# balisujohn/tortoise.cpp

Measured on AMD Instinct MI355X. Metric: audio-seconds/sec end-to-end (AR+diffusion+vocoder), 16 cands x 80 steps, higher is better.
Workload: dtype f16 MFMA inputs / f32 accumulate (diffusion, vocoder convs); f32 weights, f16 KV (AR)

## Files before the change

### tortoise.cpp_amd/csrc/api.cpp

```cpp
#include "common.h"
#include <sched.h>
#include <cctype>
#include <algorithm>
#include <chrono>
#include <fstream>
#include <new>

namespace tts {
int ar_begin(tts_ctx *, const int32_t *, int, const float *, int, int);
int ar_begin_groups(tts_ctx *, const int32_t *, const int *, int, const float *, int n_voices, const int *voice_of, const int *, int);
int ar_latents_group(tts_ctx *, int, const int32_t *, int, float *);
int ar_prefill(tts_ctx *, float *);
int ar_step(tts_ctx *, const int32_t *, int, float *, int mode);
const int32_t *ar_host_lists(tts_ctx *);
const float *ar_fetch_logits_row(tts_ctx *, int);
int ar_batch(const tts_ctx *);
int ar_latents(tts_ctx *, const int32_t *, int, int, float *);
int ar_layers(const tts_ctx *);
float *ar_host_logits(tts_ctx *);
int diff_layers(const tts_ctx *);
int diff_forward(tts_ctx *, const float *, int, const float *, int, int, float *);
int diff_sample(tts_ctx *, const float *, const int32_t *, int, int, const float *, int, float *);
int diff_sample_voices(tts_ctx *, const float *, const int32_t *, int, const float *, int, const int32_t *, int, const float *, int, float *);
int voc_run(tts_ctx *, const float *, const int32_t *, int, const float *, int, float *);
// ... 112 lines not shown
  for (hipEvent_t e : c->ev_pool) (void)hipEventDestroy(e);
  if (c->ev0) (void)hipEventDestroy(c->ev0);
  if (c->ev1) (void)hipEventDestroy(c->ev1);
  if (c->stream) (void)hipStreamDestroy(c->stream);
  if (c->load_stream) (void)hipStreamDestroy(c->load_stream);
  delete c;
}

int tts_version(void) { return TTS_API_VERSION; }

const char *tts_last_error(const tts_ctx *c) { return c ? c->err.c_str() : "no context (no HIP device?)"; }

int tts_set_option(tts_ctx *c, const char *key, double value) {
  if (!c || !key) return TTS_ERR_ARG;
  std::string k(key);
  if (k == "gn_eps") c->gn_eps = (float)value;
  else if (k == "ggml_lut") c->ggml_lut = value != 0;
  else if (k.rfind("prof_only:", 0) == 0) {
    if (value != 0) c->prof_filter.push_back(k.substr(10));
    else c->prof_filter.clear();
  }
  else if (k == "device_topk") c->device_topk = value != 0;
  else if (k == "sampler_threads") {
    if (c->sampler_pool) { sampler_pool_free(c->sampler_pool); c->sampler_pool = nullptr; }
    c->sampler_threads = value < 0 ? -1 : (int)value;
  }
  else if (k == "share_uncond") c->share_uncond = value != 0;
  else if (k == "prof_stride") c->prof_stride = value < 1 ? 1 : (int)value;
  else if (k == "diff_graph") c->diff_graph = value != 0;
  else if (k == "dec_f32_mfma") c->dec_f32_mfma = value != 0;
  else if (k == "attn_f32") c->attn_f32 = value != 0;
  else if (k == "attn_proj_f16") c->attn_proj_f16 = value != 0;
  else if (k == "proj_dual_b") c->proj_dual_b = value != 0;
  else if (k == "lc_attn_f32") c->lc_attn_f32 = value != 0;
  else if (k == "latency_mode") c->latency_mode = value != 0;
  else if (k == "fp16_check") c->fp16_check = value != 0;
  else if (k == "rng_fast_normal") c->rng_fast_normal = value != 0;
  else if (k == "noise_pipeline") c->noise_pipeline = value != 0;
  else if (k == "load_device_pack") c->load_device_pack = value != 0;
  else if (k == "load_threads") c->load_threads = value < 0 ? 0 : value > 64 ? 64 : (int)value;
  else if (k == "attn_q64") c->attn_q64 = value < 0 ? 0 : value > 2 ? 2 : (int)value;
  else if (k == "hoist_integrator") c->hoist_integrator = value < 0 ? 0 : (int)value;
  else if (k == "attn_f32_drop") c->attn_f32_drop = (int)value & 7;
  else if (k == "ar_weights") {
    if (value != 0 && value != 1 && value != 2) return fail(c, TTS_ERR_ARG, "ar_weights: 0 (f32), 1 (fp16) or 2 (fp8 e4m3)");
    c->ar_weights = (int)value;
  }
  else if (k == "prof_eager_every") c->prof_eager_every = value < 1 ? 1 : (int)value;
  else if (k == "stream_cus") {
    if (c->device < 0) return fail(c, TTS_ERR_HIP, "host-only context: no stream");
    if (c->ar || c->diff || c->voc || c->clvp || c->venc || c->dcond) return fail(c, TTS_ERR_STATE, "stream_cus must be set before the models are loaded");
    (void)hipSetDevice(c->device);
    hipDeviceProp_t prop;
    if (hipGetDeviceProperties(&prop, c->device) != hipSuccess) return fail(c, TTS_ERR_HIP, "hipGetDeviceProperties failed");
    const int xcds = 8, per_xcd = prop.multiProcessorCount / xcds, n = (int)(value < 0 ? -value : value);
    if (prop.multiProcessorCount % xcds || per_xcd > 32 || n >= per_xcd) return fail(c, TTS_ERR_ARG, "stream_cus %d: the device has %d CUs per XCD", (int)value, per_xcd);
    hipStream_t s = nullptr;
    if (n == 0) {
      if (hipStreamCreate(&s) != hipSuccess) return fail(c, TTS_ERR_HIP, "hipStreamCreate failed");
    } else {
      uint32_t mask[8] = {0, 0, 0, 0, 0, 0, 0, 0};
      for (int slot = 0; slot < per_xcd; slot++)
        if ((slot < n) == (value > 0))
          for (int x = 0; x < xcds; x++) { const int bit = slot * xcds + x; mask[bit >> 5] |= 1u << (bit & 31); }
      if (hipExtStreamCreateWithCUMask(&s, (uint32_t)((per_xcd * xcds + 31) / 32), mask) != hipSuccess)
        return fail(c, TTS_ERR_HIP, "hipExtStreamCreateWithCUMask failed");
// ... 423 lines not shown
```

### tortoise.cpp_amd/csrc/common.h

```cpp
#pragma once
#include "../../include/tortoise_mi355x.h"
#include <hip/hip_runtime.h>
#include <cstdarg>
#include <cstdint>
#include <cstdio>
#include <cstring>
#include <functional>
#include <map>
#include <memory>
#include <random>
#include <algorithm>
#include <atomic>
#include <condition_variable>
#include <mutex>
#include <new>
#include <string>
#include <thread>
#include <vector>

namespace tts {

struct HostTensor {
  std::vector<float> data;
  int64_t ne[4] = {1, 1, 1, 1};
// ... 67 lines not shown
  int device = 0;
  hipStream_t stream = nullptr;
  hipStream_t load_stream = nullptr;
  int stream_cus = 0;
  std::string err;
  float gn_eps = 1e-6f;
  int ggml_lut = 0;
  std::mt19937 generator;
  std::uniform_real_distribution<float> distribution{0.0, 1.0};
  std::normal_distribution<double> normal_distribution{0.0, 1.0};
  uint32_t seed_value = 0;
  tts::ArState *ar = nullptr;
  tts::DiffState *diff = nullptr;
  tts::VocState *voc = nullptr;
  tts::ClvpState *clvp = nullptr;
  tts::VoiceEncState *venc = nullptr;
  tts::DiffCondEncState *dcond = nullptr;
  tts::Tokenizer *tok = nullptr;
  tts::SamplerPool *sampler_pool = nullptr;
  int device_topk = 1;
  int time_mlp_retries = 0;
  int topk_fallbacks = 0;
  int sampler_threads = -1;
  bool share_uncond = true;
  int rng_shard_offset = 0, rng_shard_total = 0;
  std::vector<int32_t> stop_schedule;
  std::vector<int32_t> ar_stopped;
  bool prof_on = false;
  std::vector<std::string> prof_filter;
  int prof_stride = 1;
  int ar_weights = 0;
  int dec_f32_mfma = 0;
  int attn_f32 = 0;
  int proj_dual_b = 1;
  int attn_f32_drop = 0;
  int lc_attn_f32 = 1;
  int attn_proj_f16 = 0;
  int fp16_check = 0;
  int64_t fp16_bad_weights[2] = {0, 0};
  void *fp16_counts = nullptr;
  int rng_fast_normal = 1;
  int noise_pipeline = 1;
  int load_device_pack = 1;
  int load_threads = 0;
  int attn_q64 = 0;
  int hoist_integrator = 1;
  int latency_mode = 0;
  bool capturing = false;
  int diff_graph = 1;
  int prof_eager_every = 8;
  std::map<std::string, tts::ProfEntry> prof;
  std::vector<hipEvent_t> ev_pool;
  hipEvent_t ev0 = nullptr, ev1 = nullptr;
};

namespace tts {

int fail(tts_ctx *ctx, int code, const char *fmt, ...);

void rng_normal_fill(tts_ctx *ctx, float *dst, int64_t n);

struct PinnedPool {
  explicit PinnedPool(size_t min_cap_ = (size_t)18 << 20, int max_bufs_ = 4) : min_cap(min_cap_), max_bufs(max_bufs_) {}
  size_t min_cap;
  int max_bufs, made = 0;
  std::mutex mu;
// ... 169 lines not shown
```

### tortoise.cpp_amd/csrc/diffusion.hip

```cpp
#include "common.h"
#include "gemm_f16.h"
#include <algorithm>
#include <chrono>
#include <cmath>

namespace tts {

static constexpr int C = 1024, NHEAD = 16, XTC = 128 ;
static constexpr int LAT_MAX_ROWS = 2048;
static constexpr int HOIST_MAX_ROWS = 16384;

__device__ __forceinline__ float silu_dev(float x, int lut) {
  if (lut == 1) {
    float xr = __half2float(__float2half_rn(x));
    return __half2float(__float2half_rn(xr / (1.0f + expf(-xr))));
  }
  if (lut == 2) return x / (1.0f + expf(-x));
  return x * __builtin_amdgcn_rcpf(1.0f + __builtin_amdgcn_exp2f(x * -1.44269504088896f));
}

__global__ __launch_bounds__(256) void gn_stats_kernel(const float *__restrict__ x, const int *__restrict__ seq_start,
                                                       const int *__restrict__ seq_len, float eps, float2 *__restrict__ stats) {
  __shared__ float sh[8];
  const int grp = blockIdx.x, s = blockIdx.y, T = seq_len[s];
// ... 626 lines not shown
  {
#pragma clang fp contract(off)
    const float frac = (var_c + 1) / 2;
    model_log_variance = frac * sc.min_log + (1 - frac) * sc.max_log;
    const float eps = (1 + sc.cfk) * eps_c - sc.cfk * eps_u;
    float x0 = sc.sqrt_recip * xv - sc.sqrt_recipm1 * eps;
    x0 = fminf(fmaxf(x0, -1.0f), 1.0f);
    mean = sc.coef1 * x0 + sc.coef2 * xv;
  }
  float outv = mean;
  if (!sc.is_last) {
    const float nz = noise ? noise[xi] : philox_normal(seed, stream0 + (uint32_t)s, step, (uint32_t)(ch * T + t));
    outv = (float)((double)mean + exp(0.5 * (double)model_log_variance) * (double)nz);
  }
  x[xi] = outv;
}

__global__ void philox_fill_kernel(float *__restrict__ x, int64_t n, uint64_t seed, uint32_t stream, uint32_t step) {
  int64_t i = (int64_t)blockIdx.x * blockDim.x + threadIdx.x;
  if (i < n) x[i] = philox_normal(seed, stream, step, (uint32_t)i);
}

__global__ void rows_to_ct_kernel(const float *__restrict__ net, int row0, int T, int nch, int ld, float *__restrict__ out) {
  int i = blockIdx.x * blockDim.x + threadIdx.x;
  if (i < nch * T) {
    int ch = i / T, t = i - ch * T;
    out[i] = net[(size_t)(row0 + t) * ld + ch];
  }
}

struct AttnDev {
  float *norm_g, *norm_b, *qkv_b, *proj_b, *bias_tab;
  __half *qkv_w, *proj_w;
  __half *proj_w_split;
  float proj_alpha;
};
struct ResDev { float *in_g, *in_b, *in_bias, *emb_w, *emb_b, *out_g, *out_b, *out_bias; __half *in_w, *out_w; };

struct Layout {
  int ns = 0, rows = 0;
  std::vector<int> start, len;
  DevBuf d_row_seq, d_row_t, d_start, d_len, d_chunk_seq;
  int build(tts_ctx *ctx, const std::vector<int> &lens) {
    has_seq_step = false; ss_step_stride = 0;
    ns = (int)lens.size();
    len = lens;
    start.resize(ns);
    int r = 8;
    for (int s = 0; s < ns; s++) { start[s] = r; r = (r + lens[s] + 1 + 7) & ~7; }
    rows = (r + 127) & ~127;
    std::vector<int> rs(rows, -1), rt(rows, 0);
    for (int s = 0; s < ns; s++)
      for (int t = 0; t < lens[s]; t++) { rs[start[s] + t] = s; rt[start[s] + t] = t; }
    TTS_HIP(ctx, d_row_seq.reserve(rows * 4)); TTS_HIP(ctx, d_row_t.reserve(rows * 4));
    TTS_HIP(ctx, d_start.reserve(ns * 4)); TTS_HIP(ctx, d_len.reserve(ns * 4));
    TTS_HIP(ctx, hipMemcpy(d_row_seq.p, rs.data(), rows * 4, hipMemcpyHostToDevice));
    TTS_HIP(ctx, hipMemcpy(d_row_t.p, rt.data(), rows * 4, hipMemcpyHostToDevice));
    TTS_HIP(ctx, hipMemcpy(d_start.p, start.data(), ns * 4, hipMemcpyHostToDevice));
    TTS_HIP(ctx, hipMemcpy(d_len.p, len.data(), ns * 4, hipMemcpyHostToDevice));
    std::vector<int> cs(rows / 8, -1);
    for (int s = 0; s < ns; s++)
      for (int t = 0; t < lens[s]; t++) cs[(start[s] + t) >> 3] = s;
    TTS_HIP(ctx, d_chunk_seq.reserve(rows / 8 * 4));
    TTS_HIP(ctx, hipMemcpy(d_chunk_seq.p, cs.data(), rows / 8 * 4, hipMemcpyHostToDevice));
    return TTS_OK;
  }
  int max_len() const { return len.empty() ? 0 : *std::max_element(len.begin(), len.end()); }
  DevBuf d_seq_step;
  int ss_step_stride = 0;
  bool has_seq_step = false;
// ... 87 lines not shown
  if (!latent2048) return fail(ctx, TTS_ERR_ARG, "null latent");
  TTS_HIP(ctx, hipMemcpyAsync(ctx->diff->cond_latent, latent2048, (size_t)2 * C * 4, hipMemcpyHostToDevice, ctx->stream));
  TTS_HIP(ctx, hipStreamSynchronize(ctx->stream));
  return TTS_OK;
}

namespace {
struct Loader {
  tts_ctx *ctx; DiffState *st; const WeightFile &wf; std::map<std::string, bool> used; std::mutex mu; PinnedPool pin{(size_t)9 << 20, 4};
  const HostTensor *get(const std::string &name, int64_t nelem) {
    auto it = wf.t.find(name);
    if (it == wf.t.end()) { fail(ctx, TTS_ERR_FORMAT, "tensor '%s' missing from diffusion model file", name.c_str()); return nullptr; }
    if (it->second.nelem() != nelem) {
      fail(ctx, TTS_ERR_FORMAT, "tensor '%s' has wrong size in model file: got %lld, expected %lld", name.c_str(),
           (long long)it->second.nelem(), (long long)nelem);
      return nullptr;
    }
    { std::lock_guard<std::mutex> lk(mu); used[name] = true; }
    return &it->second;
  }
  template <class T> int put(const std::vector<T> &h, T **dst) {
    void *p = nullptr;
    TTS_HIP(ctx, hipMalloc(&p, h.size() * sizeof(T)));
    { std::lock_guard<std::mutex> lk(mu); st->owned.push_back(p); }
    TTS_HIP(ctx, pin.upload(p, h.data(), h.size() * sizeof(T), ctx->load_stream));
    *dst = (T *)p;
    return TTS_OK;
  }
  int f32(const std::string &name, int64_t n, float **dst) {
    const HostTensor *t = get(name, n);
    if (!t) return TTS_ERR_FORMAT;
    return put(t->data, dst);
  }
  int conv16(const std::string &name, int cout, int cin, int k, int cout_pad, int cin_pad, __half **dst) {
    const HostTensor *t = get(name, (int64_t)cout * cin * k);
    if (!t) return TTS_ERR_FORMAT;
    std::vector<__half> h((size_t)cout_pad * k * cin_pad, __float2half(0.f));
    const float *w = t->data.data();
    for (int co = 0; co < cout; co++)
      for (int ci = 0; ci < cin; ci++)
        for (int tap = 0; tap < k; tap++)
          h[(size_t)co * k * cin_pad + (size_t)tap * cin_pad + ci] = __float2half_rn(w[((size_t)co * cin + ci) * k + tap]);
    return put(h, dst);
  }
  int attn(const std::string &p, AttnDev &a) {
    int r;
    if ((r = f32(p + ".norm.weight", C, &a.norm_g))) return r;
    if ((r = f32(p + ".norm.bias", C, &a.norm_b))) return r;
    if ((r = conv16(p + ".qkv.weight", 3 * C, C, 1, 3 * C, C, &a.qkv_w))) return r;
    if ((r = f32(p + ".qkv.bias", 3 * C, &a.qkv_b))) return r;
    if ((r = conv16(p + ".proj_out.weight", C, C, 1, C, C, &a.proj_w))) return r;
    {
      const HostTensor *t = get(p + ".proj_out.weight", (int64_t)C * C);
      std::vector<__half> sp((size_t)C * 2 * C);
      float amax = 0.f;
      for (float v : t->data) amax = std::max(amax, std::fabs(v));
      if (!std::isfinite(amax)) { fail(ctx, TTS_ERR_FORMAT, "tensor '%s.proj_out.weight' holds a non-finite value", p.c_str()); return TTS_ERR_FORMAT; }
      int e = 14;
      while (e > -14 && std::ldexp(amax, e) >= 30000.0f) e--;
      const float scale = std::ldexp(1.0f, e);
      a.proj_alpha = 1.0f / scale;
      for (int n = 0; n < C; n++)
        for (int k = 0; k < C; k++) {
          const float w = t->data[(size_t)n * C + k] * scale;
          const __half hi = __float2half_rn(w);
          sp[(size_t)n * 2 * C + k] = hi;
          sp[(size_t)n * 2 * C + C + k] = __float2half_rn(w - __half2float(hi));
        }
      long long bad[2] = {0, 0};
      for (const __half &h : sp) {
        const float v = std::fabs(__half2float(h));
        if (!(v <= 65504.0f)) bad[0]++;
        else if (v > 60000.0f) bad[1]++;
      }
      if (bad[0] | bad[1]) { std::lock_guard<std::mutex> lk(mu); ctx->fp16_bad_weights[0] += bad[0]; ctx->fp16_bad_weights[1] += bad[1]; }
      if ((r = put(sp, &a.proj_w_split))) return r;
    }
    if ((r = f32(p + ".proj_out.bias", C, &a.proj_b))) return r;
    const HostTensor *t = get(p + ".relative_pos_embeddings.relative_attention_bias.weight", 32 * 16);
    if (!t) return TTS_ERR_FORMAT;
    std::vector<float> tab(16 * 128);
    for (int h = 0; h < 16; h++)
      for (int sgn = 0; sgn < 2; sgn++)
        for (int d = 0; d < 64; d++) {
          int bucket = sgn ? rel_bucket(0, d) : rel_bucket(d, 0);
          if (d == 0) bucket = rel_bucket(0, 0);
          tab[h * 128 + sgn * 64 + d] = t->data[(size_t)bucket * 16 + h] * 8.0f;
        }
    return put(tab, &a.bias_tab);
  }
  int res(const std::string &p, ResDev &w) {
    int r;
    if ((r = f32(p + ".in_layers.0.weight", C, &w.in_g))) return r;
    if ((r = f32(p + ".in_layers.0.bias", C, &w.in_b))) return r;
    if ((r = conv16(p + ".in_layers.2.weight", C, C, 1, C, C, &w.in_w))) return r;
    if ((r = f32(p + ".in_layers.2.bias", C, &w.in_bias))) return r;
    if ((r = f32(p + ".emb_layers.1.weight", 2 * C * C, &w.emb_w))) return r;
    if ((r = f32(p + ".emb_layers.1.bias", 2 * C, &w.emb_b))) return r;
    if ((r = f32(p + ".out_layers.0.weight", C, &w.out_g))) return r;
    if ((r = f32(p + ".out_layers.0.bias", C, &w.out_b))) return r;
    if ((r = conv16(p + ".out_layers.3.weight", C, C, 3, C, C, &w.out_w))) return r;
    if ((r = f32(p + ".out_layers.3.bias", C, &w.out_bias))) return r;
    return TTS_OK;
  }
};
}

int diff_load(tts_ctx *ctx, const char *path) {
  ctx->fp16_bad_weights[0] = ctx->fp16_bad_weights[1] = 0;
  WeightFile wf;
  std::string err;
  int rc = read_weight_file(path, wf, err);
  if (rc != TTS_OK) return fail(ctx, rc, "diffusion_model_load: %s", err.c_str());
  std::unique_ptr<DiffState> st(new DiffState());
  Loader ld{ctx, st.get(), wf, {}};
  while (wf.has("latent_conditioner." + std::to_string(st->n_lc + 1) + ".norm.weight")) st->n_lc++;
  while (wf.has("conditioning_timestep_integrator." + std::to_string(st->n_integ) + ".resblk.in_layers.0.weight")) st->n_integ++;
  while (wf.has("layers." + std::to_string(st->n_main) + ".resblk.in_layers.0.weight")) st->n_main++;
  while (wf.has("layers." + std::to_string(st->n_main + st->n_tail) + ".in_layers.0.weight")) st->n_tail++;
  st->lc_attn.resize(st->n_lc);
  st->integ_res.resize(st->n_integ); st->integ_attn.resize(st->n_integ);
  st->main_res.resize(st->n_main); st->main_attn.resize(st->n_main);
  st->tail_res.resize(st->n_tail);
  std::vector<std::function<int()>> jobs;
  DiffState *S = st.get();
#define J(x) jobs.emplace_back([&ld, S]() -> int { (void)S; return (x); })
  J(ld.f32("diffusion_conditioning_latent", 2 * C, &S->cond_latent));
  J(ld.f32("unconditioned_embedding", C, &S->uncond_emb));
// ... 77 lines not shown
  int64_t dev[2] = {0, 0};
  if (ctx->fp16_counts) {
    TTS_HIP(ctx, hipStreamSynchronize(ctx->stream));
    TTS_HIP(ctx, hipMemcpy(dev, ctx->fp16_counts, 16, hipMemcpyDeviceToHost));
  }
  counts[0] = dev[0] + ctx->fp16_bad_weights[0];
  counts[1] = dev[1] + ctx->fp16_bad_weights[1];
  return TTS_OK;
}

static int gemm(tts_ctx *ctx, const char *fam, GemmArgs &g, const Layout &lay, int n_valid = 0, int k_valid = 0) {
  double mv = 0;
  for (int l : lay.len) mv += l;
  static const bool log_shapes = getenv("TTS_GEMM_LOG") != nullptr;
  if (log_shapes) fprintf(stderr, "gemm M=%d N=%d K=%dx%d mode=%d resid=%d\n", g.M, g.N, g.nseg, g.kseg, g.mode, g.resid != nullptr);
  if (!strcmp(fam, "diff_gemm")) {
    if (g.mode == GEMM_OUT_QKV) fam = "diff_gemm_qkv";
    else if (gemm_is_conv3(g) && g.N == C && g.kseg == C) fam = g.resid ? "diff_gemm_k3r" : "diff_gemm_k3";
    else if (g.nseg == 1 && g.N == C && g.kseg == C && g.mode == GEMM_OUT_F32) fam = g.resid ? "diff_gemm_k1r" : "diff_gemm_k1";
    else if (g.custom_w && g.N == C && g.kseg == C && g.mode == GEMM_OUT_F32_SCALED && g.resid) fam = "diff_gemm_k1r";
    else fam = "diff_gemm_misc";
  }
  ProfScope ps(ctx, fam, 2.0 * mv * (n_valid ? n_valid : g.N) * (k_valid ? k_valid : g.nseg * g.kseg));
  TTS_HIP(ctx, launch_gemm_f16(g, ctx->stream));
  if (ctx->fp16_check) {
    if (gemm_mode_qkv(g.mode)) {
      CHECK(fp16_check(ctx, g.outH, (size_t)g.M * g.ldh));
      CHECK(fp16_check(ctx, g.outVt, (size_t)(g.N / 3) * g.ldvt));
    } else if (g.mode == GEMM_OUT_F16) CHECK(fp16_check(ctx, g.outH, (size_t)g.M * g.ldh));
  }
  return TTS_OK;
}

static GemmArgs gemm_base(const Layout &lay, const __half *A, int lda, int nseg, int kseg, const __half *W, int N,
                          const float *bias) {
  GemmArgs g{};
  for (int i = 0; i < 3; i++) { g.A[i] = A; g.row_off[i] = 0; }
  if (nseg == 3) { g.row_off[0] = -1; g.row_off[1] = 0; g.row_off[2] = 1; }
  g.nseg = nseg; g.kseg = kseg; g.lda = lda; g.W = W; g.M = lay.rows; g.N = N; g.bias = bias;
  g.row_seq = lay.d_row_seq.as<int>();
  return g;
}

static int gn_stats(tts_ctx *ctx, const Layout &lay, Work &wk, const float *x) {
  ProfScope ps(ctx, "diff_gn_stats");
  gn_stats_kernel<<<dim3(32, lay.ns), 256, 0, ctx->stream>>>(x, lay.d_start.as<int>(), lay.d_len.as<int>(), ctx->gn_eps,
                                                             wk.stats.as<float2>());
  TTS_HIP(ctx, hipGetLastError());
  return TTS_OK;
}
template <int NT, int NJ>
__global__ __launch_bounds__(NT) void gn_reg_kernel(const float *__restrict__ x, const int *__restrict__ seq_start,
                                                    const int *__restrict__ seq_len, int rows_total, int ns, float eps,
                                                    const float *__restrict__ g, const float *__restrict__ b,
                                                    const float *__restrict__ ss, int do_silu, int lut, __half *__restrict__ y,
                                                    const char *__restrict__ pf0, int pf0_lines, const char *__restrict__ pf1, int pf1_lines,
                                                    const int *__restrict__ seq_step, int ss_step_stride) {
  constexpr int NW = NT / 64, SWEEP = NT / 8;
  __shared__ float sh[2][NW];
  __shared__ unsigned pf_sink[NW][64];
  const int bid = blockIdx.y * 32 + blockIdx.x, nbk = ns * 32, item = (bid & 7) * (nbk >> 3) + (bid >> 3);
  const int s = item >> 5, grp = item & 31;
  const int T = seq_len[s], r0 = seq_start[s];
  const int q = threadIdx.x & 7, c = grp * 32 + q * 4, t0 = threadIdx.x >> 3;
  const float *base = x + (size_t)r0 * C + c;
  float4 v[NJ];
// ... 157 lines not shown
      const __half2 p0 = __floats2half2_rn(e[0], e[1]), p1 = __floats2half2_rn(e[2], e[3]);
      uint2 o;
      o.x = *(const unsigned *)&p0;
      o.y = *(const unsigned *)&p1;
      *(uint2 *)(y + (size_t)(r0 + r) * C + c) = o;
    }
  };
  if (!do_silu) apply(std::integral_constant<int, 0>{});
  else if (lut == 0) apply(std::integral_constant<int, 1>{});
  else if (lut == 1) apply(std::integral_constant<int, 2>{});
  else apply(std::integral_constant<int, 3>{});
  if (pf0_lines | pf1_lines) asm volatile("s_waitcnt vmcnt(0)" ::: "memory");
}

static int gn(tts_ctx *ctx, const DiffState *st, const Layout &lay, const float *x, const long long *st_x, const float *g, const float *b, const float *ss, int do_silu,
              __half *y, const void *wa = nullptr, size_t wa_bytes = 0, const void *wb = nullptr, size_t wb_bytes = 0) {
  if (!st_x) {
    CHECK(gn_fused(ctx, lay, x, g, b, ss, do_silu, y, wa, wa_bytes, wb, wb_bytes));
    return fp16_check(ctx, y, (size_t)lay.rows * C);
  }
  {
    ProfScope ps(ctx, "diff_gn_apply");
    const int silu_mode = ctx->ggml_lut ? 1 : ctx->attn_f32 ? 2 : 0;
    gn_apply_kernel<<<lay.rows / 4, 256, 0, ctx->stream>>>(x, lay.d_chunk_seq.as<int>(), lay.d_start.as<int>(), lay.d_len.as<int>(), st_x, (int)st->gn_stripe_ll, ctx->gn_eps, g, b,
                                                            ss, do_silu, silu_mode, y, (const char *)wa, (int)(wa_bytes >> 7), (const char *)wb, (int)(wb_bytes >> 7),
                                                            lay.seq_step_ptr(), lay.ss_step_stride);
    TTS_HIP(ctx, hipGetLastError());
  }
  return fp16_check(ctx, y, (size_t)lay.rows * C);
}

static int res_in_layers(tts_ctx *ctx, const DiffState *st, const Layout &lay, Work &wk, const float *x, const ResDev &w, float *H,
                         const long long *st_x = nullptr, long long *st_h_out = nullptr) {
  CHECK(gn(ctx, st, lay, x, st_x, w.in_g, w.in_b, nullptr, 1, wk.A16(), w.in_w, (size_t)C * C * 2));
  DBG_SUM("res.in gn", wk.A16(), (size_t)lay.rows * C * 2);
  GemmArgs g = gemm_base(lay, wk.A16(), C, 1, C, w.in_w, C, w.in_bias);
  g.mode = st_h_out ? GEMM_OUT_F32_STATS : GEMM_OUT_F32; g.outF = H; g.ldo = C; g.resid = nullptr;
  g.st_out = st_h_out; g.st_stripe_ll = (int)st->gn_stripe_ll; g.chunk_seq = lay.d_chunk_seq.as<int>();
  CHECK(gemm(ctx, "diff_gemm", g, lay));
  DBG_SUM("res.in conv", H, (size_t)lay.rows * C * 4);
  return TTS_OK;
}

static int attention_block(tts_ctx *ctx, DiffState *st, const Layout &lay, Work &wk, float *X, const AttnDev &w, bool force_ref = false) {
  const bool f32 = ctx->attn_f32 != 0 || force_ref;
  const bool pw16 = !f32 && ctx->attn_proj_f16;
  const bool lat = st->lat && wk.st_x != nullptr;
  CHECK(gn(ctx, st, lay, X, lat ? wk.st_x : nullptr, w.norm_g, w.norm_b, nullptr, 0, wk.A16(), w.qkv_w, (size_t)3 * C * C * 2, pw16 ? w.proj_w : w.proj_w_split,
           (size_t)C * C * (pw16 ? 2 : 4)));
  long long *st_out = lat ? st->new_stats_slot() : nullptr;
  wk.st_x = st_out;
  DBG_SUM("attn gn", wk.A16(), (size_t)lay.rows * C * 2);
  GemmArgs g = gemm_base(lay, wk.A16(), C, 1, C, w.qkv_w, 3 * C, w.qkv_b);
  g.mode = f32 ? GEMM_OUT_QKV_SPLIT : GEMM_OUT_QKV;
  g.outH = wk.qk16.as<__half>(); g.ldh = 2048; g.outVt = wk.vt16.as<__half>(); g.ldvt = wk.rows + 128;
  g.outH2 = wk.qk16_lo.as<__half>(); g.outVt2 = wk.vt16_lo.as<__half>();
  CHECK(gemm(ctx, "diff_gemm", g, lay));
  if (f32 && (ctx->attn_f32_drop & 1)) TTS_HIP(ctx, hipMemsetAsync(wk.qk16_lo.p, 0, (size_t)(wk.rows + 128) * 2048 * 2, ctx->stream));
  if (f32 && (ctx->attn_f32_drop & 2)) TTS_HIP(ctx, hipMemsetAsync(wk.vt16_lo.p, 0, (size_t)C * (wk.rows + 128) * 2, ctx->stream));
  DBG_SUM("attn qk", wk.qk16.p, (size_t)lay.rows * 2048 * 2);
  DBG_SUM("attn vt", wk.vt16.p, (size_t)C * (wk.rows + 128) * 2);
  {
    double aw = 0;
    for (int l : lay.len) aw += 4.0 * l * (double)l * 64 * NHEAD;
    ProfScope ps(ctx, "diff_attn", aw);
    const int nq = (lay.max_len() + 127) / 128;
    if (f32) {
      diff_attn_f32_kernel<<<nq * NHEAD * lay.ns, 256, ATT32_LDS, ctx->stream>>>(wk.qk16.as<__half>(), wk.qk16_lo.as<__half>(), wk.vt16.as<__half>(),
                                                                                 wk.vt16_lo.as<__half>(), wk.rows + 128, lay.d_start.as<int>(),
                                                                                 lay.d_len.as<int>(), w.bias_tab, wk.ATT16(), wk.att16_lo.as<__half>() + C, nq);
    } else {
      const bool q64 = ctx->attn_q64 == 1 || (ctx->attn_q64 == 2 && nq * NHEAD * lay.ns <= 256);
      if (q64) {
        const int nq64 = (lay.max_len() + 63) / 64;
        diff_attn_kernel<2, 1><<<nq64 * NHEAD * lay.ns, 256, att_lds<2>(), ctx->stream>>>(wk.qk16.as<__half>(), wk.vt16.as<__half>(), wk.rows + 128,
                                                                                      lay.d_start.as<int>(), lay.d_len.as<int>(), w.bias_tab, wk.ATT16(), nq64);
      } else
        diff_attn_kernel<2, 2><<<nq * NHEAD * lay.ns, 256, att_lds<2>(), ctx->stream>>>(wk.qk16.as<__half>(), wk.vt16.as<__half>(), wk.rows + 128,
                                                                                    lay.d_start.as<int>(), lay.d_len.as<int>(), w.bias_tab, wk.ATT16(), nq);
    }
    TTS_HIP(ctx, hipGetLastError());
  }
  CHECK(fp16_check(ctx, wk.ATT16(), (size_t)lay.rows * C));
  if (f32 && (ctx->attn_f32_drop & 4)) TTS_HIP(ctx, hipMemsetAsync(wk.att16_lo.p, 0, (size_t)(wk.rows + 2) * C * 2, ctx->stream));
  DBG_SUM("attn out", wk.ATT16(), (size_t)lay.rows * C * 2);
  if (f32) {
    GemmArgs p = gemm_base(lay, wk.ATT16(), C, 3, C, w.proj_w_split, C, w.proj_b);
// ... 559 lines not shown
```

### tortoise.cpp_amd/csrc/gemm_f16.h

```cpp
#pragma once
#include <hip/hip_fp16.h>
#include <hip/hip_runtime.h>
#include <algorithm>
#include <cmath>
#include <cstdlib>
#include <type_traits>

namespace tts {

typedef _Float16 half8 __attribute__((ext_vector_type(8)));
typedef float floatx4 __attribute__((ext_vector_type(4)));

enum { GEMM_OUT_F32 = 0, GEMM_OUT_F16 = 1, GEMM_OUT_QKV = 2, GEMM_OUT_QKV_SPLIT = 3, GEMM_OUT_F32_SCALED = 4, GEMM_OUT_F32_STATS = 5, GEMM_OUT_F32_SCALED_STATS = 6 };
constexpr bool gemm_mode_qkv(int mode) { return mode == GEMM_OUT_QKV || mode == GEMM_OUT_QKV_SPLIT; }
constexpr bool gemm_mode_f32(int mode) { return mode == GEMM_OUT_F32 || mode == GEMM_OUT_F32_SCALED || mode == GEMM_OUT_F32_STATS || mode == GEMM_OUT_F32_SCALED_STATS; }
constexpr bool gemm_mode_scaled(int mode) { return mode == GEMM_OUT_F32_SCALED || mode == GEMM_OUT_F32_SCALED_STATS; }
constexpr bool gemm_mode_stats(int mode) { return mode == GEMM_OUT_F32_STATS || mode == GEMM_OUT_F32_SCALED_STATS; }

struct GemmArgs {
  const __half *A[3];
  int row_off[3];
  int nseg, kseg;
  int lda;
  const __half *W;
  int ldw_, w_off_[3], custom_w;
  int M, N;
  const float *bias;
  const int *row_seq;
  float *outF; int ldo; const float *resid;
  __half *outH; int ldh;
  __half *outVt; int ldvt;
  __half *outH2, *outVt2;
  float alpha;
  long long *st_out;
  int st_stripe_ll;
  const int *chunk_seq;
  int dual_b;
  int mode;
  int th, cn;
  int ku;
  const int4 *tiles; int tab_len;
};


__device__ __forceinline__ int lds_swz(int row) { return ((row >> 1) & 3) << 1; }
__device__ __forceinline__ int lds_off(int row, int chunk) { return row * 128 + ((chunk ^ lds_swz(row)) << 4); }

typedef const void __attribute__((address_space(1))) *gptr_t;
typedef void __attribute__((address_space(3))) *lptr_t;

__device__ __forceinline__ int vh_blk(int wm, int i) { return wm + 2 * i; }

__device__ __forceinline__ float split_lo(float x) { return x - __half2float(__float2half_rn(x)); }
__device__ __forceinline__ uint2 pack_half4(float a, float b, float c, float d) {
  const __half2 p0 = __floats2half2_rn(a, b), p1 = __floats2half2_rn(c, d);
  uint2 u;
  u.x = *(const unsigned *)&p0;
  u.y = *(const unsigned *)&p1;
// ... 390 lines not shown
  m0 = blk0 << 4;
  nblk = min(g.th, b1 - blk0);
  n0 = (chunk * g.cn + rem - t * g.cn) << 7;
  return true;
}

static constexpr int GEMM_VH_LDS = 32768;
template <int MODE, int WGS, int KU = 1>
static __global__ __launch_bounds__(256, WGS) void gemm_f16_vh_kernel(GemmArgs g) {
  const int tid = threadIdx.x, lane = tid & 63, wave = __builtin_amdgcn_readfirstlane(tid >> 6);
  int m0, n0, nblk;
  if (!gemm_vh_tile(g, m0, n0, nblk)) return;
  const int my_mi = (nblk - (wave >> 1) + 1) >> 1;
  if (my_mi == 4) gemm_vh_body<MODE, 4, KU>(g, m0, n0, nblk, lane, wave);
  else if (my_mi == 3) gemm_vh_body<MODE, 3, KU>(g, m0, n0, nblk, lane, wave);
  else if (my_mi == 2) gemm_vh_body<MODE, 2, KU>(g, m0, n0, nblk, lane, wave);
  else if (my_mi == 1) gemm_vh_body<MODE, 1, KU>(g, m0, n0, nblk, lane, wave);
  else gemm_vh_body<MODE, 0, KU>(g, m0, n0, nblk, lane, wave);
}

template <int MODE, int KU = 1>
static __global__ __launch_bounds__(256, KU == 1 ? 3 : 1) void gemm_f16_vh_dualb_kernel(GemmArgs g) {
  const int tid = threadIdx.x, lane = tid & 63, wave = __builtin_amdgcn_readfirstlane(tid >> 6);
  int m0, n0, nblk;
  if (!gemm_vh_tile(g, m0, n0, nblk)) return;
  const int my_mi = (nblk - (wave >> 1) + 1) >> 1;
  if (my_mi == 4) gemm_vh_dualb_body<MODE, 4, KU>(g, m0, n0, nblk, lane, wave);
  else if (my_mi == 3) gemm_vh_dualb_body<MODE, 3, KU>(g, m0, n0, nblk, lane, wave);
  else if (my_mi == 2) gemm_vh_dualb_body<MODE, 2, KU>(g, m0, n0, nblk, lane, wave);
  else if (my_mi == 1) gemm_vh_dualb_body<MODE, 1, KU>(g, m0, n0, nblk, lane, wave);
  else gemm_vh_dualb_body<MODE, 0, KU>(g, m0, n0, nblk, lane, wave);
}

static constexpr int CONV3_VH_LDS = (128 + 8) * 128 + 2 * 16384;
template <int MODE, int MI>
__device__ __forceinline__ void gemm_conv3_vh_body(const GemmArgs &g, int m0, int n0, int nblk, int lane, int wave) {
  extern __shared__ __attribute__((aligned(16))) char smem_dyn[];
  char *smem = smem_dyn;
  constexpr int MA = MI > 0 ? MI : 1;
  const int wm = wave >> 1, wn = wave & 1;
  const int my_pa = (2 * nblk + 1 - wave + 3) >> 2;
  const int nchunks = g.kseg >> 6, ldw = 3 * g.kseg, nph = 3 * nchunks;
  const int prow = lane >> 3, pslot = lane & 7;
  const int fr = lane & 15, fq = lane >> 4;
  floatx4 acc[MA][4];
#pragma unroll
  for (int i = 0; i < MI; i++)
#pragma unroll
    for (int j = 0; j < 4; j++) acc[i][j] = (floatx4){0.f, 0.f, 0.f, 0.f};
  char *sa = smem, *sb = smem + (128 + 8) * 128;
  const __half *abase = g.A[0] + (ptrdiff_t)(m0 - 1) * g.lda;
  const __half *wbase = g.W + (size_t)n0 * ldw;
  int aoff[5], boff[4];
#pragma unroll
  for (int i = 0; i < 5; i++) {
    const int row = (wave + 4 * i) * 8 + prow;
    aoff[i] = min(row, g.M - m0 + 1) * g.lda + (pslot ^ lds_swz(row)) * 8;
  }
#pragma unroll
  for (int i = 0; i < 4; i++) {
    const int row = (wave * 4 + i) * 8 + prow;
    boff[i] = row * ldw + (pslot ^ lds_swz(row)) * 8;
  }
  auto stageA = [&](int kc) {
    const __half *src = abase + (min(kc, nchunks - 1) << 6);
#pragma unroll
// ... 31 lines not shown
    asm volatile("s_waitcnt lgkmcnt(0)" ::: "memory");
    __builtin_amdgcn_s_barrier();
    if (TAP == 2) stageA(kc + 1);
  };
  stageA(0);
  stageB(0);
  for (int kc = 0; kc < nchunks; kc++) {
    const int p = 3 * kc;
    phase(kc, p, std::integral_constant<int, 0>{});
    phase(kc, p + 1, std::integral_constant<int, 1>{});
    phase(kc, p + 2, std::integral_constant<int, 2>{});
  }
  asm volatile("s_waitcnt vmcnt(0)" ::: "memory");
  if ((MODE == GEMM_OUT_F32 || MODE == GEMM_OUT_F32_STATS) && g.resid) gemm_epilogue_vh<MODE, MI, EPI_RESID_LOAD>(g, acc, m0, n0, wm, wn, fr, fq);
  else gemm_epilogue_vh<MODE, MI, EPI_NO_RESID>(g, acc, m0, n0, wm, wn, fr, fq);
}

template <int MODE>
static __global__ __launch_bounds__(256, 3) void gemm_f16_conv3_vh_kernel(GemmArgs g) {
  const int tid = threadIdx.x, lane = tid & 63, wave = __builtin_amdgcn_readfirstlane(tid >> 6);
  int m0, n0, nblk;
  if (!gemm_vh_tile(g, m0, n0, nblk)) return;
  const int my_mi = (nblk - (wave >> 1) + 1) >> 1;
  if (my_mi == 4) gemm_conv3_vh_body<MODE, 4>(g, m0, n0, nblk, lane, wave);
  else if (my_mi == 3) gemm_conv3_vh_body<MODE, 3>(g, m0, n0, nblk, lane, wave);
  else if (my_mi == 2) gemm_conv3_vh_body<MODE, 2>(g, m0, n0, nblk, lane, wave);
  else if (my_mi == 1) gemm_conv3_vh_body<MODE, 1>(g, m0, n0, nblk, lane, wave);
  else gemm_conv3_vh_body<MODE, 0>(g, m0, n0, nblk, lane, wave);
}

static inline bool gemm_is_conv3(const GemmArgs &g) {
  return g.nseg == 3 && !g.custom_w && g.A[0] == g.A[1] && g.A[1] == g.A[2] && g.row_off[0] == -1 && g.row_off[1] == 0 && g.row_off[2] == 1 &&
         !gemm_mode_qkv(g.mode) && !gemm_mode_scaled(g.mode);
}

static inline hipError_t launch_gemm_f16(const GemmArgs &g, hipStream_t s) {
  GemmArgs gg = g;
  const int NT = g.N >> 7, ktot = g.nseg * g.kseg, nb = g.M >> 4;
  if (gemm_mode_scaled(g.mode)) {
    int e;
    if (!(g.alpha != 0.f) || std::fabs(std::frexp(g.alpha, &e)) != 0.5f) return hipErrorInvalidValue;
  }
  if (gemm_mode_stats(g.mode) && (!g.st_out || !g.chunk_seq || g.st_stripe_ll <= 0)) return hipErrorInvalidValue;
  if (g.dual_b && !(gemm_mode_scaled(g.mode) && g.nseg == 2 && g.custom_w && g.A[0] == g.A[1] && g.row_off[0] == g.row_off[1])) return hipErrorInvalidValue;
  int ku = (g.ku == 2 || g.ku == 4) && (g.kseg % (64 * g.ku)) == 0 ? g.ku : 1;
  int grid;
  if (g.tiles) grid = 8 * g.tab_len;
  else {
    int cn = NT;
    if (NT > 8)
      for (cn = NT; cn > 1; cn--)
        if (NT % cn == 0 && (size_t)cn * 128 * ktot * 2 <= (size_t)2560 * 1024) break;
    gg.cn = cn;
    const int maxb = (nb + 7) / 8 + 1;
    auto tiles_at = [&](int h) { return 8 * ((maxb + h - 1) / h) * NT; };
    int th = g.th;
    if (th <= 0) { th = 2; while (th < 8 && tiles_at(th) > 1024) th *= 2; }
    if (g.th <= 0 && g.ku == 0 && NT <= 8 && tiles_at(4) <= 256 && (g.kseg % 256) == 0) {
      th = 4;
      if (!gemm_is_conv3(g)) ku = g.dual_b ? 2 : 4;
    }
    gg.th = th;
    int mt_max = 0;
    for (int x = 0; x < 8; x++) {
      const int b0 = (int)((long long)nb * x >> 3), b1 = (int)((long long)nb * (x + 1) >> 3);
      mt_max = std::max(mt_max, (b1 - b0 + th - 1) / th);
    }
    grid = 8 * mt_max * NT;
  }
  if (gemm_is_conv3(g)) {
    static bool attr = false;
    if (!attr) {
      (void)hipFuncSetAttribute((const void *)gemm_f16_conv3_vh_kernel<GEMM_OUT_F32>, hipFuncAttributeMaxDynamicSharedMemorySize, CONV3_VH_LDS);
      (void)hipFuncSetAttribute((const void *)gemm_f16_conv3_vh_kernel<GEMM_OUT_F32_STATS>, hipFuncAttributeMaxDynamicSharedMemorySize, CONV3_VH_LDS);
      (void)hipFuncSetAttribute((const void *)gemm_f16_conv3_vh_kernel<GEMM_OUT_F16>, hipFuncAttributeMaxDynamicSharedMemorySize, CONV3_VH_LDS);
      attr = true;
    }
    if (g.mode == GEMM_OUT_F32) gemm_f16_conv3_vh_kernel<GEMM_OUT_F32><<<grid, 256, CONV3_VH_LDS, s>>>(gg);
    else if (g.mode == GEMM_OUT_F32_STATS) gemm_f16_conv3_vh_kernel<GEMM_OUT_F32_STATS><<<grid, 256, CONV3_VH_LDS, s>>>(gg);
    else gemm_f16_conv3_vh_kernel<GEMM_OUT_F16><<<grid, 256, CONV3_VH_LDS, s>>>(gg);
  } else if (g.dual_b && gemm_mode_scaled(g.mode) && g.nseg == 2 && g.custom_w && g.A[0] == g.A[1] && g.row_off[0] == g.row_off[1]) {
#define TTS_DUALB_LAUNCH(MODE_)                                                                                                                     \
  do {                                                                                                                                              \
    if (ku == 2) {                                                                                                                                  \
      static bool a2 = false;                                                                                                                       \
      if (!a2) { (void)hipFuncSetAttribute((const void *)gemm_f16_vh_dualb_kernel<MODE_, 2>, hipFuncAttributeMaxDynamicSharedMemorySize, 2 * GEMM_DUALB_LDS); a2 = true; } \
      gemm_f16_vh_dualb_kernel<MODE_, 2><<<grid, 256, 2 * GEMM_DUALB_LDS, s>>>(gg);                                                                  \
    } else gemm_f16_vh_dualb_kernel<MODE_, 1><<<grid, 256, GEMM_DUALB_LDS, s>>>(gg);                                                                \
  } while (0)
    if (g.mode == GEMM_OUT_F32_SCALED) TTS_DUALB_LAUNCH(GEMM_OUT_F32_SCALED);
    else TTS_DUALB_LAUNCH(GEMM_OUT_F32_SCALED_STATS);
#undef TTS_DUALB_LAUNCH
  } else {
#define TTS_VH_LAUNCH(MODE_)                                                                                                                      \
  do {                                                                                                                                            \
    if (ku == 1) gemm_f16_vh_kernel<MODE_, 4><<<grid, 256, GEMM_VH_LDS, s>>>(gg);                                                                 \
    else if (ku == 2) {                                                                                                                           \
      static bool a2 = false;                                                                                                                     \
      if (!a2) { (void)hipFuncSetAttribute((const void *)gemm_f16_vh_kernel<MODE_, 2, 2>, hipFuncAttributeMaxDynamicSharedMemorySize, 2 * GEMM_VH_LDS); a2 = true; } \
      gemm_f16_vh_kernel<MODE_, 2, 2><<<grid, 256, 2 * GEMM_VH_LDS, s>>>(gg);                                                                     \
    } else {                                                                                                                                      \
      static bool a4 = false;                                                                                                                     \
      if (!a4) { (void)hipFuncSetAttribute((const void *)gemm_f16_vh_kernel<MODE_, 1, 4>, hipFuncAttributeMaxDynamicSharedMemorySize, 4 * GEMM_VH_LDS); a4 = true; } \
// ... 17 lines not shown
```

Measured before the change: 134.6.

## Add register-resident fragment-layout weight GEMM path for diffusion 1x1 convs

Adds a new GEMM kernel for the diffusion model's ResBlock input conv and attention QKV projection. At load time it pre-arranges the weights into an MFMA fragment layout, so each wave loads its weight fragments straight from global memory into registers. Only the activation tile goes through LDS, cutting LDS traffic and footprint. The path is on by default when the auto tile height is 8, and it costs a second copy of those weights plus a new kernel with inline asm waitcnt scheduling.

```diff
diff --git a/tortoise.cpp_amd/csrc/api.cpp b/tortoise.cpp_amd/csrc/api.cpp
--- a/tortoise.cpp_amd/csrc/api.cpp
+++ b/tortoise.cpp_amd/csrc/api.cpp
@@ -168,6 +168,7 @@
   else if (k == "attn_f32") c->attn_f32 = value != 0;
   else if (k == "attn_proj_f16") c->attn_proj_f16 = value != 0;
   else if (k == "proj_dual_b") c->proj_dual_b = value != 0;
+  else if (k == "gemm_wreg") c->gemm_wreg = value == 1 ? tts_ctx::GEMM_WREG_ALL : value == 2 ? 1 : value == 3 ? 2 : 0;
   else if (k == "lc_attn_f32") c->lc_attn_f32 = value != 0;
   else if (k == "latency_mode") c->latency_mode = value != 0;
   else if (k == "fp16_check") c->fp16_check = value != 0;
diff --git a/tortoise.cpp_amd/csrc/common.h b/tortoise.cpp_amd/csrc/common.h
--- a/tortoise.cpp_amd/csrc/common.h
+++ b/tortoise.cpp_amd/csrc/common.h
@@ -123,6 +123,8 @@
   int ar_weights = 0;
   int dec_f32_mfma = 0;
   int attn_f32 = 0;
+  static constexpr int GEMM_WREG_ALL = 3;
+  int gemm_wreg = GEMM_WREG_ALL;
   int proj_dual_b = 1;
   int attn_f32_drop = 0;
   int lc_attn_f32 = 1;
diff --git a/tortoise.cpp_amd/csrc/diffusion.hip b/tortoise.cpp_amd/csrc/diffusion.hip
--- a/tortoise.cpp_amd/csrc/diffusion.hip
+++ b/tortoise.cpp_amd/csrc/diffusion.hip
@@ -682,10 +682,11 @@
 struct AttnDev {
   float *norm_g, *norm_b, *qkv_b, *proj_b, *bias_tab;
   __half *qkv_w, *proj_w;
+  __half *qkv_wf;
   __half *proj_w_split;
   float proj_alpha;
 };
-struct ResDev { float *in_g, *in_b, *in_bias, *emb_w, *emb_b, *out_g, *out_b, *out_bias; __half *in_w, *out_w; };
+struct ResDev { float *in_g, *in_b, *in_bias, *emb_w, *emb_b, *out_g, *out_b, *out_bias; __half *in_w, *out_w, *in_wf; };
 
 struct Layout {
   int ns = 0, rows = 0;
@@ -839,7 +840,7 @@
     if (!t) return TTS_ERR_FORMAT;
     return put(t->data, dst);
   }
-  int conv16(const std::string &name, int cout, int cin, int k, int cout_pad, int cin_pad, __half **dst) {
+  int conv16(const std::string &name, int cout, int cin, int k, int cout_pad, int cin_pad, __half **dst, __half **dst_frag = nullptr) {
     const HostTensor *t = get(name, (int64_t)cout * cin * k);
     if (!t) return TTS_ERR_FORMAT;
     std::vector<__half> h((size_t)cout_pad * k * cin_pad, __float2half(0.f));
@@ -848,13 +849,19 @@
       for (int ci = 0; ci < cin; ci++)
         for (int tap = 0; tap < k; tap++)
           h[(size_t)co * k * cin_pad + (size_t)tap * cin_pad + ci] = __float2half_rn(w[((size_t)co * cin + ci) * k + tap]);
+    if (dst_frag) {
+      std::vector<__half> f(h.size());
+      for (int n = 0; n < cout_pad; n++)
+        for (int c = 0; c < cin_pad; c++) f[gemm_wfrag_index(n, c, cin_pad)] = h[(size_t)n * cin_pad + c];
+      if (int r = put(f, dst_frag)) return r;
+    }
     return put(h, dst);
   }
   int attn(const std::string &p, AttnDev &a) {
     int r;
     if ((r = f32(p + ".norm.weight", C, &a.norm_g))) return r;
     if ((r = f32(p + ".norm.bias", C, &a.norm_b))) return r;
-    if ((r = conv16(p + ".qkv.weight", 3 * C, C, 1, 3 * C, C, &a.qkv_w))) return r;
+    if ((r = conv16(p + ".qkv.weight", 3 * C, C, 1, 3 * C, C, &a.qkv_w, &a.qkv_wf))) return r;
     if ((r = f32(p + ".qkv.bias", 3 * C, &a.qkv_b))) return r;
     if ((r = conv16(p + ".proj_out.weight", C, C, 1, C, C, &a.proj_w))) return r;
     {
@@ -900,7 +907,7 @@
     int r;
     if ((r = f32(p + ".in_layers.0.weight", C, &w.in_g))) return r;
     if ((r = f32(p + ".in_layers.0.bias", C, &w.in_b))) return r;
-    if ((r = conv16(p + ".in_layers.2.weight", C, C, 1, C, C, &w.in_w))) return r;
+    if ((r = conv16(p + ".in_layers.2.weight", C, C, 1, C, C, &w.in_w, &w.in_wf))) return r;
     if ((r = f32(p + ".in_layers.2.bias", C, &w.in_bias))) return r;
     if ((r = f32(p + ".emb_layers.1.weight", 2 * C * C, &w.emb_w))) return r;
     if ((r = f32(p + ".emb_layers.1.bias", 2 * C, &w.emb_b))) return r;
@@ -1044,6 +1051,11 @@
   return TTS_OK;
 }
 
+static int gemm_wreg_class(const tts_ctx *ctx, int bit) { return (ctx->gemm_wreg & bit) ? 1 : 0; }
+static const __half *gemm_wreg_image(const tts_ctx *ctx, int bit, const Layout &lay, int N, const __half *w, const __half *wf) {
+  return gemm_wreg_class(ctx, bit) && gemm_auto_th(lay.rows, N) == 8 ? wf : w;
+}
+
 static GemmArgs gemm_base(const Layout &lay, const __half *A, int lda, int nseg, int kseg, const __half *W, int N,
                           const float *bias) {
   GemmArgs g{};
@@ -1267,10 +1279,11 @@
 
 static int res_in_layers(tts_ctx *ctx, const DiffState *st, const Layout &lay, Work &wk, const float *x, const ResDev &w, float *H,
                          const long long *st_x = nullptr, long long *st_h_out = nullptr) {
-  CHECK(gn(ctx, st, lay, x, st_x, w.in_g, w.in_b, nullptr, 1, wk.A16(), w.in_w, (size_t)C * C * 2));
+  CHECK(gn(ctx, st, lay, x, st_x, w.in_g, w.in_b, nullptr, 1, wk.A16(), gemm_wreg_image(ctx, 1, lay, C, w.in_w, w.in_wf), (size_t)C * C * 2));
   DBG_SUM("res.in gn", wk.A16(), (size_t)lay.rows * C * 2);
   GemmArgs g = gemm_base(lay, wk.A16(), C, 1, C, w.in_w, C, w.in_bias);
   g.mode = st_h_out ? GEMM_OUT_F32_STATS : GEMM_OUT_F32; g.outF = H; g.ldo = C; g.resid = nullptr;
+  g.Wf = w.in_wf; g.wreg = gemm_wreg_class(ctx, 1);
   g.st_out = st_h_out; g.st_stripe_ll = (int)st->gn_stripe_ll; g.chunk_seq = lay.d_chunk_seq.as<int>();
   CHECK(gemm(ctx, "diff_gemm", g, lay));
   DBG_SUM("res.in conv", H, (size_t)lay.rows * C * 4);
@@ -1281,13 +1294,14 @@
   const bool f32 = ctx->attn_f32 != 0 || force_ref;
   const bool pw16 = !f32 && ctx->attn_proj_f16;
   const bool lat = st->lat && wk.st_x != nullptr;
-  CHECK(gn(ctx, st, lay, X, lat ? wk.st_x : nullptr, w.norm_g, w.norm_b, nullptr, 0, wk.A16(), w.qkv_w, (size_t)3 * C * C * 2, pw16 ? w.proj_w : w.proj_w_split,
+  CHECK(gn(ctx, st, lay, X, lat ? wk.st_x : nullptr, w.norm_g, w.norm_b, nullptr, 0, wk.A16(), gemm_wreg_image(ctx, 2, lay, 3 * C, w.qkv_w, w.qkv_wf), (size_t)3 * C * C * 2, pw16 ? w.proj_w : w.proj_w_split,
            (size_t)C * C * (pw16 ? 2 : 4)));
   long long *st_out = lat ? st->new_stats_slot() : nullptr;
   wk.st_x = st_out;
   DBG_SUM("attn gn", wk.A16(), (size_t)lay.rows * C * 2);
   GemmArgs g = gemm_base(lay, wk.A16(), C, 1, C, w.qkv_w, 3 * C, w.qkv_b);
   g.mode = f32 ? GEMM_OUT_QKV_SPLIT : GEMM_OUT_QKV;
+  g.Wf = w.qkv_wf; g.wreg = gemm_wreg_class(ctx, 2);
   g.outH = wk.qk16.as<__half>(); g.ldh = 2048; g.outVt = wk.vt16.as<__half>(); g.ldvt = wk.rows + 128;
   g.outH2 = wk.qk16_lo.as<__half>(); g.outVt2 = wk.vt16_lo.as<__half>();
   CHECK(gemm(ctx, "diff_gemm", g, lay));
diff --git a/tortoise.cpp_amd/csrc/gemm_f16.h b/tortoise.cpp_amd/csrc/gemm_f16.h
--- a/tortoise.cpp_amd/csrc/gemm_f16.h
+++ b/tortoise.cpp_amd/csrc/gemm_f16.h
@@ -24,6 +24,8 @@
   int lda;
   const __half *W;
   int ldw_, w_off_[3], custom_w;
+  const __half *Wf;
+  int wreg;
   int M, N;
   const float *bias;
   const int *row_seq;
@@ -480,6 +482,215 @@
   else gemm_vh_dualb_body<MODE, 0, KU>(g, m0, n0, nblk, lane, wave);
 }
 
+static inline size_t gemm_wfrag_index(int n, int k, int K) {
+  return ((((size_t)(n >> 4) * (K >> 5) + (k >> 5)) * 64 + ((k >> 3) & 3) * 16 + (n & 15)) << 3) + (k & 7);
+}
+
+template <int OFF> __device__ __forceinline__ void wreg_load(half8 &d, const __half *base, unsigned voff) {
+  asm volatile("global_load_dwordx4 %0, %1, %2 offset:%3" : "=v"(d) : "v"(voff), "s"(base), "i"(OFF));
+}
+template <int N> __device__ __forceinline__ void wreg_wait(half8 &a, half8 &b, half8 &c, half8 &d) {
+  asm volatile("s_waitcnt vmcnt(%4)" : "+v"(a), "+v"(b), "+v"(c), "+v"(d) : "i"(N) : "memory");
+}
+
+template <int MODE, int MI, bool NAT>
+__device__ __forceinline__ void gemm_epilogue_wreg(const GemmArgs &g, floatx4 (&acc)[MI][2], int m0, int n0, int nblk, int wave, int fr, int fq) {
+  const int c0 = n0 + wave * 32;
+  const bool hb = g.bias != nullptr, hs = g.row_seq != nullptr;
+  const float *bp = hb ? g.bias : (const float *)g.W;
+  const int *sp = hs ? g.row_seq : (const int *)g.A[0];
+  if (NAT) {
+    const int h = c0 / 192, w0 = c0 - h * 192;
+    {
+      float bv[2];
+      int4 sq[MI];
+#pragma unroll
+      for (int j = 0; j < 2; j++) bv[j] = bp[c0 + j * 16 + fr];
+#pragma unroll
+      for (int i = 0; i < MI; i++) sq[i] = *(const int4 *)(sp + m0 + min(i, nblk - 1) * 16 + fq * 4);
+#pragma unroll
+      for (int j = 0; j < 2; j++) bv[j] = hb ? bv[j] : 0.f;
+#pragma unroll
+      for (int i = 0; i < MI; i++) sq[i] = hs ? sq[i] : make_int4(0, 0, 0, 0);
+#pragma unroll
+      for (int i = 0; i < MI; i++) {
+        if (i < nblk) {
+          const int rbase = m0 + i * 16 + fq * 4;
+          const bool gd[4] = {sq[i].x < 0, sq[i].y < 0, sq[i].z < 0, sq[i].w < 0};
+#pragma unroll
+          for (int j = 0; j < 2; j++) {
+            float v[4];
+#pragma unroll
+            for (int r = 0; r < 4; r++) v[r] = gd[r] ? 0.f : acc[i][j][r] + bv[j];
+            const size_t o = (size_t)(h * 64 + (w0 - 128) + j * 16 + fr) * g.ldvt + rbase;
+            *(uint2 *)(g.outVt + o) = pack_half4(v[0], v[1], v[2], v[3]);
+            if (MODE == GEMM_OUT_QKV_SPLIT) *(uint2 *)(g.outVt2 + o) = pack_half4(split_lo(v[0]), split_lo(v[1]), split_lo(v[2]), split_lo(v[3]));
+          }
+        }
+      }
+      return;
+    }
+  }
+  const int col0 = c0 + fq * 4;
+  float4 b4[2];
+  int sq[MI];
+#pragma unroll
+  for (int j = 0; j < 2; j++) b4[j] = *(const float4 *)(bp + col0 + j * 16);
+#pragma unroll
+  for (int i = 0; i < MI; i++) sq[i] = sp[m0 + min(i, nblk - 1) * 16 + fr];
+#pragma unroll
+  for (int j = 0; j < 2; j++) b4[j] = hb ? b4[j] : make_float4(0.f, 0.f, 0.f, 0.f);
+#pragma unroll
+  for (int i = 0; i < MI; i++) sq[i] = hs ? sq[i] : 0;
+  auto finish = [&](int i, int j) {
+    float4 v = make_float4(acc[i][j][0] + b4[j].x, acc[i][j][1] + b4[j].y, acc[i][j][2] + b4[j].z, acc[i][j][3] + b4[j].w);
+    if (sq[i] < 0) v = make_float4(0.f, 0.f, 0.f, 0.f);
+    return v;
+  };
+  if (MODE == GEMM_OUT_F32) {
+#pragma unroll
+    for (int i = 0; i < MI; i++) {
+      if (i < nblk) {
+        float *op = g.outF + (size_t)(m0 + i * 16 + fr) * g.ldo + col0;
+#pragma unroll
+        for (int j = 0; j < 2; j++) *(float4 *)(op + j * 16) = finish(i, j);
+      }
+    }
+  } else {
+    const int h = c0 / 192, w0 = c0 - h * 192;
+#pragma unroll
+    for (int i = 0; i < MI; i++) {
+      if (i < nblk) {
+        __half *op = g.outH + (size_t)(m0 + i * 16 + fr) * g.ldh + h * 128 + w0 + fq * 4;
+#pragma unroll
+        for (int j = 0; j < 2; j++) {
+          const float4 v = finish(i, j);
+          *(uint2 *)(op + j * 16) = pack_half4(v.x, v.y, v.z, v.w);
+          if (MODE == GEMM_OUT_QKV_SPLIT)
+            *(uint2 *)(g.outH2 + (op - g.outH) + j * 16) = pack_half4(split_lo(v.x), split_lo(v.y), split_lo(v.z), split_lo(v.w));
+        }
+      }
+    }
+  }
+}
+
+template <int MODE, int MI, int D, bool NAT>
+__device__ __forceinline__ void gemm_wreg_body(const GemmArgs &g, int m0, int n0, int nblk, int lane, int wave) {
+  extern __shared__ __attribute__((aligned(16))) char smem_dyn[];
+  char *smem = smem_dyn;
+  constexpr int S = D + 1;
+  constexpr int NPA = MI / 2;
+  constexpr int PER = NPA + 4;
+  static_assert(D == 1 || D == 2, "prefetch distance");
+  const int T = g.kseg >> 6, KS = g.kseg >> 5;
+  const int prow = lane >> 3, pslot = lane & 7;
+  const int fr = lane & 15, fq = lane >> 4;
+  unsigned aoff[NPA];
+#pragma unroll
+  for (int i = 0; i < NPA; i++) {
+    const int row = (wave + 4 * i) * 8 + prow;
+    aoff[i] = (unsigned)((min(row, nblk * 16 - 1) * g.lda + (pslot ^ lds_swz(row)) * 8) * 2);
+  }
+  const char *aseg = (const char *)(g.A[0] + (ptrdiff_t)(g.row_off[0] + m0) * g.lda);
+  const __half *wp0 = g.Wf + (size_t)((n0 >> 4) + wave * 2) * KS * 512, *wp1 = wp0 + (size_t)KS * 512;
+  const unsigned wlane = lane * 16;
+  const bool resid_first = MODE == GEMM_OUT_F32 && g.resid != nullptr;
+  floatx4 acc[MI][2];
+  if (resid_first) {
+#pragma unroll
+    for (int i = 0; i < MI; i++) {
+      const int row = m0 + min(i, nblk - 1) * 16 + fr;
+#pragma unroll
+      for (int j = 0; j < 2; j++) {
+        const float4 rr = *(const float4 *)(g.resid + (size_t)row * g.ldo + n0 + wave * 32 + j * 16 + fq * 4);
+        acc[i][j] = (floatx4){rr.x, rr.y, rr.z, rr.w};
+      }
+    }
+  } else {
+#pragma unroll
+    for (int i = 0; i < MI; i++)
+#pragma unroll
+      for (int j = 0; j < 2; j++) acc[i][j] = (floatx4){0.f, 0.f, 0.f, 0.f};
+  }
+  half8 w[S][2][2];
+  auto issue = [&](int t, auto set_c) {
+    constexpr int U = decltype(set_c)::value;
+    const char *ab = aseg + (t << 7);
+#pragma unroll
+    for (int i = 0; i < NPA; i++) __builtin_amdgcn_global_load_lds((gptr_t)(ab + aoff[i]), (lptr_t)(smem + U * 16384 + (wave + 4 * i) * 1024), 16, 0, 0);
+    const __half *q0 = wp0 + (size_t)t * 1024, *q1 = wp1 + (size_t)t * 1024;
+    wreg_load<0>(w[U][0][0], q0, wlane);
+    wreg_load<0>(w[U][0][1], q1, wlane);
+    wreg_load<1024>(w[U][1][0], q0, wlane);
+    wreg_load<1024>(w[U][1][1], q1, wlane);
+  };
+  auto kloop = [&]() {
+    auto step = [&](int t, auto u_c) {
+      constexpr int U = decltype(u_c)::value;
+      if (D == 2 && t + 1 < T) wreg_wait<PER>(w[U][0][0], w[U][0][1], w[U][1][0], w[U][1][1]);
+      else wreg_wait<0>(w[U][0][0], w[U][0][1], w[U][1][0], w[U][1][1]);
+      asm volatile("s_waitcnt lgkmcnt(0)" ::: "memory");
+      __builtin_amdgcn_s_barrier();
+      if (t + D < T) issue(t + D, std::integral_constant<int, (U + D) % S>{});
+      const char *sa = smem + U * 16384;
+      constexpr int AHEAD = 2;
+      half8 af[AHEAD + 1];
+      auto frag = [&](int x) { return *(const half8 *)(sa + lds_off((x % MI) * 16 + fr, (x / MI) * 4 + fq)); };
+#pragma unroll
+      for (int x = 0; x < AHEAD; x++) af[x] = frag(x);
+#pragma unroll
+      for (int x = 0; x < 2 * MI; x++) {
+        if (x + AHEAD < 2 * MI) af[(x + AHEAD) % (AHEAD + 1)] = frag(x + AHEAD);
+        const int ks = x / MI, i = x % MI;
+        const half8 a = af[x % (AHEAD + 1)];
+#pragma unroll
+        for (int j = 0; j < 2; j++) {
+          if (NAT) acc[i][j] = __builtin_amdgcn_mfma_f32_16x16x32_f16(a, w[U][ks][j], acc[i][j], 0, 0, 0);
+          else acc[i][j] = __builtin_amdgcn_mfma_f32_16x16x32_f16(w[U][ks][j], a, acc[i][j], 0, 0, 0);
+        }
+      }
+      __builtin_amdgcn_sched_group_barrier(0x100, AHEAD, 0);
+#pragma unroll
+      for (int x = 0; x < 2 * MI; x++) {
+        if (x + AHEAD < 2 * MI) __builtin_amdgcn_sched_group_barrier(0x100, 1, 0);
+        __builtin_amdgcn_sched_group_barrier(0x008, 2, 0);
+      }
+    };
+    for (int t0 = 0; t0 < T; t0 += S) {
+      step(t0, std::integral_constant<int, 0>{});
+      if (t0 + 1 < T) step(t0 + 1, std::integral_constant<int, 1>{});
+      if (S == 3 && t0 + 2 < T) step(t0 + 2, std::integral_constant<int, S - 1>{});
+    }
+  };
+  issue(0, std::integral_constant<int, 0>{});
+  if (D == 2) issue(1, std::integral_constant<int, 1>{});
+#pragma unroll
+  for (int i = 0; i < MI; i++)
+#pragma unroll
+    for (int j = 0; j < 2; j++) asm volatile("" : "+v"(acc[i][j]));
+  kloop();
+  gemm_epilogue_wreg<MODE, MI, NAT>(g, acc, m0, n0, nblk, wave, fr, fq);
+}
+
+static constexpr int GEMM_WREG_D = 1, GEMM_WREG_LDS = (GEMM_WREG_D + 1) * 16384;
+template <int MODE, int D = GEMM_WREG_D>
+static __global__ __launch_bounds__(256, 4) void gemm_f16_wreg_kernel(GemmArgs g) {
+  const int tid = threadIdx.x, lane = tid & 63, wave = __builtin_amdgcn_readfirstlane(tid >> 6);
+  int m0, n0, nblk;
+  if (!gemm_vh_tile(g, m0, n0, nblk)) return;
+  if (gemm_mode_qkv(MODE) && ((n0 + wave * 32) % 192) >= 128) {
+    if (nblk > 4) gemm_wreg_body<MODE, 8, D, true>(g, m0, n0, nblk, lane, wave);
+    else gemm_wreg_body<MODE, 4, D, true>(g, m0, n0, nblk, lane, wave);
+  } else {
+    if (nblk > 4) gemm_wreg_body<MODE, 8, D, false>(g, m0, n0, nblk, lane, wave);
+    else gemm_wreg_body<MODE, 4, D, false>(g, m0, n0, nblk, lane, wave);
+  }
+}
+static inline bool gemm_takes_wreg(const GemmArgs &g, int th, int ku) {
+  return g.wreg > 0 && g.Wf && !g.tiles && g.nseg == 1 && !g.custom_w && th == 8 && ku == 1 && (g.kseg >> 6) >= 2 &&
+         (g.mode == GEMM_OUT_F32 || g.mode == GEMM_OUT_QKV || g.mode == GEMM_OUT_QKV_SPLIT);
+}
+
 static constexpr int CONV3_VH_LDS = (128 + 8) * 128 + 2 * 16384;
 template <int MODE, int MI>
 __device__ __forceinline__ void gemm_conv3_vh_body(const GemmArgs &g, int m0, int n0, int nblk, int lane, int wave) {
@@ -577,6 +788,13 @@
 static inline bool gemm_is_conv3(const GemmArgs &g) {
   return g.nseg == 3 && !g.custom_w && g.A[0] == g.A[1] && g.A[1] == g.A[2] && g.row_off[0] == -1 && g.row_off[1] == 0 && g.row_off[2] == 1 &&
          !gemm_mode_qkv(g.mode) && !gemm_mode_scaled(g.mode);
+}
+
+static inline int gemm_auto_th(int M, int N) {
+  const int maxb = ((M >> 4) + 7) / 8 + 1, NT = N >> 7;
+  int th = 2;
+  while (th < 8 && 8 * ((maxb + th - 1) / th) * NT > 1024) th *= 2;
+  return th;
 }
 
 static inline hipError_t launch_gemm_f16(const GemmArgs &g, hipStream_t s) {
@@ -600,7 +818,7 @@
     const int maxb = (nb + 7) / 8 + 1;
     auto tiles_at = [&](int h) { return 8 * ((maxb + h - 1) / h) * NT; };
     int th = g.th;
-    if (th <= 0) { th = 2; while (th < 8 && tiles_at(th) > 1024) th *= 2; }
+    if (th <= 0) th = gemm_auto_th(g.M, g.N);
     if (g.th <= 0 && g.ku == 0 && NT <= 8 && tiles_at(4) <= 256 && (g.kseg % 256) == 0) {
       th = 4;
       if (!gemm_is_conv3(g)) ku = g.dual_b ? 2 : 4;
@@ -613,7 +831,11 @@
     }
     grid = 8 * mt_max * NT;
   }
-  if (gemm_is_conv3(g)) {
+  if (gemm_takes_wreg(g, gg.th, ku)) {
+    if (g.mode == GEMM_OUT_F32) gemm_f16_wreg_kernel<GEMM_OUT_F32><<<grid, 256, GEMM_WREG_LDS, s>>>(gg);
+    else if (g.mode == GEMM_OUT_QKV) gemm_f16_wreg_kernel<GEMM_OUT_QKV><<<grid, 256, GEMM_WREG_LDS, s>>>(gg);
+    else gemm_f16_wreg_kernel<GEMM_OUT_QKV_SPLIT><<<grid, 256, GEMM_WREG_LDS, s>>>(gg);
+  } else if (gemm_is_conv3(g)) {
     static bool attr = false;
     if (!attr) {
       (void)hipFuncSetAttribute((const void *)gemm_f16_conv3_vh_kernel<GEMM_OUT_F32>, hipFuncAttributeMaxDynamicSharedMemorySize, CONV3_VH_LDS);
```

Result: faster. 136.6 (median of 6 runs) (+1.5%).
